# Kaixhin/imitation-learning

Hardware: NVIDIA H100
Metric: env_steps_per_s (higher is better)
Workload: dtype f32

## Files before the change

imitation-learning_b200/csrc/tc_gemm.cu:

```cuda
#include "common.cuh"
#include <cstdio>
#include <cstdlib>

namespace {

constexpr int BM = 128, BN = 256, BK = 16;
constexpr int THREADS = 256;
constexpr int A_BYTES = BM * BK * 4, B_BYTES = BN * BK * 4;
constexpr int A_HI = 0, A_LO = A_BYTES, B_HI = 2 * A_BYTES, B_LO = 2 * A_BYTES + B_BYTES;
constexpr int STAGE_BYTES = 2 * (A_BYTES + B_BYTES);
constexpr int N_STAGES = 3;
constexpr int RAW_STAGES = 3;
constexpr int HEAD_MAX = 8;
constexpr int HEAD_BYTES = (BN + HEAD_MAX * BN) * 4;
constexpr int L1_MAXK = 16, L1_ROWS = 256;
constexpr int L1_W_BYTES = L1_ROWS * L1_MAXK * 4, L1_B_BYTES = L1_ROWS * 4, L1_X_BYTES = BM * L1_MAXK * 4;
constexpr int raw_a_bytes(bool fuse) { return fuse ? 0 : A_BYTES; }
constexpr int raw_bytes(bool fuse) { return raw_a_bytes(fuse) + B_BYTES; }
constexpr int RAW_OFF = N_STAGES * STAGE_BYTES;
constexpr int head_off(bool fuse) { return RAW_OFF + RAW_STAGES * raw_bytes(fuse); }
constexpr int l1_off(bool fuse) { return head_off(fuse) + HEAD_BYTES; }
constexpr int smem_bytes(bool fuse) { return 1024 + l1_off(fuse) + (fuse ? L1_W_BYTES + L1_B_BYTES + L1_X_BYTES : 0); }
static_assert(smem_bytes(false) <= 227 * 1024 && smem_bytes(true) <= 227 * 1024, "tc_gemm: shared memory over the 227 KB per-CTA limit");

__device__ __forceinline__ uint32_t smem_u32(const void* p) { return (uint32_t)__cvta_generic_to_shared(p); }
__device__ __forceinline__ void fence_proxy_async() { asm volatile("fence.proxy.async.shared::cta;" ::: "memory"); }
__device__ __forceinline__ void wgmma_fence() { asm volatile("wgmma.fence.sync.aligned;" ::: "memory"); }
__device__ __forceinline__ void wgmma_commit() { asm volatile("wgmma.commit_group.sync.aligned;" ::: "memory"); }
template <int N>
__device__ __forceinline__ void wgmma_wait() { asm volatile("wgmma.wait_group.sync.aligned %0;" ::"n"(N) : "memory"); }
__device__ __forceinline__ void cp_async16(uint32_t dst, const float* src) { asm volatile("cp.async.cg.shared.global [%0], [%1], 16;" ::"r"(dst), "l"(src) : "memory"); }
__device__ __forceinline__ void cp_async_commit() { asm volatile("cp.async.commit_group;" ::: "memory"); }
template <int N>
__device__ __forceinline__ void cp_async_wait() { asm volatile("cp.async.wait_group %0;" ::"n"(N) : "memory"); }
__device__ __forceinline__ void wgmma_tf32(float (&d)[128], uint64_t a_desc, uint64_t b_desc) {
  asm volatile(
      "wgmma.mma_async.sync.aligned.m64n256k8.f32.tf32.tf32 {"
      "%0, %1, %2, %3, %4, %5, %6, %7, %8, %9, %10, %11, %12, %13, %14, %15, "
      "%16, %17, %18, %19, %20, %21, %22, %23, %24, %25, %26, %27, %28, %29, %30, %31, "
      "%32, %33, %34, %35, %36, %37, %38, %39, %40, %41, %42, %43, %44, %45, %46, %47, "
      "%48, %49, %50, %51, %52, %53, %54, %55, %56, %57, %58, %59, %60, %61, %62, %63, "
      "%64, %65, %66, %67, %68, %69, %70, %71, %72, %73, %74, %75, %76, %77, %78, %79, "
      "%80, %81, %82, %83, %84, %85, %86, %87, %88, %89, %90, %91, %92, %93, %94, %95, "
      "%96, %97, %98, %99, %100, %101, %102, %103, %104, %105, %106, %107, %108, %109, %110, %111, "
      "%112, %113, %114, %115, %116, %117, %118, %119, %120, %121, %122, %123, %124, %125, %126, %127 "
      "}, %128, %129, 1, 1, 1;"
      : "+f"(d[0]), "+f"(d[1]), "+f"(d[2]), "+f"(d[3]), "+f"(d[4]), "+f"(d[5]), "+f"(d[6]), "+f"(d[7]),
        "+f"(d[8]), "+f"(d[9]), "+f"(d[10]), "+f"(d[11]), "+f"(d[12]), "+f"(d[13]), "+f"(d[14]), "+f"(d[15]),
        "+f"(d[16]), "+f"(d[17]), "+f"(d[18]), "+f"(d[19]), "+f"(d[20]), "+f"(d[21]), "+f"(d[22]), "+f"(d[23]),
        "+f"(d[24]), "+f"(d[25]), "+f"(d[26]), "+f"(d[27]), "+f"(d[28]), "+f"(d[29]), "+f"(d[30]), "+f"(d[31]),
        "+f"(d[32]), "+f"(d[33]), "+f"(d[34]), "+f"(d[35]), "+f"(d[36]), "+f"(d[37]), "+f"(d[38]), "+f"(d[39]),
        "+f"(d[40]), "+f"(d[41]), "+f"(d[42]), "+f"(d[43]), "+f"(d[44]), "+f"(d[45]), "+f"(d[46]), "+f"(d[47]),
        "+f"(d[48]), "+f"(d[49]), "+f"(d[50]), "+f"(d[51]), "+f"(d[52]), "+f"(d[53]), "+f"(d[54]), "+f"(d[55]),
        "+f"(d[56]), "+f"(d[57]), "+f"(d[58]), "+f"(d[59]), "+f"(d[60]), "+f"(d[61]), "+f"(d[62]), "+f"(d[63]),
        "+f"(d[64]), "+f"(d[65]), "+f"(d[66]), "+f"(d[67]), "+f"(d[68]), "+f"(d[69]), "+f"(d[70]), "+f"(d[71]),
        "+f"(d[72]), "+f"(d[73]), "+f"(d[74]), "+f"(d[75]), "+f"(d[76]), "+f"(d[77]), "+f"(d[78]), "+f"(d[79]),
        "+f"(d[80]), "+f"(d[81]), "+f"(d[82]), "+f"(d[83]), "+f"(d[84]), "+f"(d[85]), "+f"(d[86]), "+f"(d[87]),
        "+f"(d[88]), "+f"(d[89]), "+f"(d[90]), "+f"(d[91]), "+f"(d[92]), "+f"(d[93]), "+f"(d[94]), "+f"(d[95]),
        "+f"(d[96]), "+f"(d[97]), "+f"(d[98]), "+f"(d[99]), "+f"(d[100]), "+f"(d[101]), "+f"(d[102]), "+f"(d[103]),
        "+f"(d[104]), "+f"(d[105]), "+f"(d[106]), "+f"(d[107]), "+f"(d[108]), "+f"(d[109]), "+f"(d[110]), "+f"(d[111]),
        "+f"(d[112]), "+f"(d[113]), "+f"(d[114]), "+f"(d[115]), "+f"(d[116]), "+f"(d[117]), "+f"(d[118]), "+f"(d[119]),
        "+f"(d[120]), "+f"(d[121]), "+f"(d[122]), "+f"(d[123]), "+f"(d[124]), "+f"(d[125]), "+f"(d[126]), "+f"(d[127])
      : "l"(a_desc), "l"(b_desc));
}
__device__ __forceinline__ uint64_t make_desc(uint32_t smem_addr) {
  return (uint64_t)((smem_addr >> 4) & 0x3FFF) | ((uint64_t)1 << 16) | ((uint64_t)(512 >> 4) << 32) | ((uint64_t)2 << 62);
}
__device__ __forceinline__ uint32_t sw64(int r, int c) { return (uint32_t)((r >> 3) * 512 + (r & 7) * 64 + ((c ^ ((r >> 1) & 3)) << 4)); }
__device__ __forceinline__ void sts128(uint32_t addr, uint32_t x, uint32_t y, uint32_t z, uint32_t w) {
  asm volatile("st.shared.v4.b32 [%0], {%1, %2, %3, %4};" ::"r"(addr), "r"(x), "r"(y), "r"(z), "r"(w) : "memory");
}
__device__ __forceinline__ uint4 lds128(uint32_t addr) {
  uint4 v;
  asm volatile("ld.shared.v4.b32 {%0, %1, %2, %3}, [%4];" : "=r"(v.x), "=r"(v.y), "=r"(v.z), "=r"(v.w) : "r"(addr));
  return v;
}
__device__ __forceinline__ uint32_t hi_of(uint32_t x) { return x & 0xFFFFE000u; }
__device__ __forceinline__ uint32_t lo_of(uint32_t x) { return __float_as_uint(__uint_as_float(x) - __uint_as_float(x & 0xFFFFE000u)); }
__device__ __forceinline__ void store_chunk(uint32_t hi_tile, uint32_t lo_tile, uint32_t off, uint4 v, bool split) {
  sts128(hi_tile + off, hi_of(v.x), hi_of(v.y), hi_of(v.z), hi_of(v.w));
  if (split) sts128(lo_tile + off, lo_of(v.x), lo_of(v.y), lo_of(v.z), lo_of(v.w));
}
__device__ __forceinline__ void store_block_t(uint32_t hi_tile, uint32_t lo_tile, int c4, int kg, const uint4 (&v)[4], bool split) {
  uint4 q0 = make_uint4(v[0].x, v[1].x, v[2].x, v[3].x), q1 = make_uint4(v[0].y, v[1].y, v[2].y, v[3].y);
  uint4 q2 = make_uint4(v[0].z, v[1].z, v[2].z, v[3].z), q3 = make_uint4(v[0].w, v[1].w, v[2].w, v[3].w);
  const int s = (c4 >> 1) & 3;
  if (s & 1) { const uint4 t = q0; q0 = q1; q1 = q2; q2 = q3; q3 = t; }
  if (s & 2) { uint4 t = q0; q0 = q2; q2 = t; t = q1; q1 = q3; q3 = t; }
  store_chunk(hi_tile, lo_tile, sw64(4 * c4 + (s & 3), kg), q0, split);
  store_chunk(hi_tile, lo_tile, sw64(4 * c4 + ((s + 1) & 3), kg), q1, split);
  store_chunk(hi_tile, lo_tile, sw64(4 * c4 + ((s + 2) & 3), kg), q2, split);
  store_chunk(hi_tile, lo_tile, sw64(4 * c4 + ((s + 3) & 3), kg), q3, split);
}

struct TcParams {
  GemmArgs g;
  int tiles_m;
  int split;
  const float* head_w;
  const float* head_b;
  float* head_out;
  int64_t head_gs, head_out_gs;
  int head_n, store_c;
  int head_js, head_ns;
  TcFuseL1 l1;
};

template <int EPI, bool FUSE = false>
__global__ void __launch_bounds__(THREADS, 1) tc_gemm_kernel(const TcParams p) {
  extern __shared__ uint8_t smem_raw[];
  uint8_t* smem = reinterpret_cast<uint8_t*>((reinterpret_cast<uintptr_t>(smem_raw) + 1023) & ~(uintptr_t)1023);
  float* head_s = reinterpret_cast<float*>(smem + head_off(FUSE));
  const uint32_t stage0 = smem_u32(smem), raw0 = stage0 + RAW_OFF;
  const uint32_t w1s = stage0 + l1_off(FUSE), b1s = w1s + L1_W_BYTES, xs = b1s + L1_B_BYTES;
  constexpr uint32_t RAW_A = 0, RAW_B = raw_a_bytes(FUSE), RAW_BYTES = raw_bytes(FUSE);

  const int tid = threadIdx.x, warp = tid >> 5, lane = tid & 31, wg = tid >> 7;
  const GemmArgs& g = p.g;
  const int nkb = g.K / BK, tiles_m = p.tiles_m;
  const int my_tiles = (g.G * tiles_m - (int)blockIdx.x + (int)gridDim.x - 1) / (int)gridDim.x;
  const int nq = my_tiles * nkb;
  const bool a_km = FUSE || g.a_kmajor != 0, b_km = g.b_kmajor != 0, split = p.split != 0;

  const int fr = tid >> 2, fc = tid & 3;
  const int a_c4 = tid & 31, a_kg = (tid >> 5) & 3, b_c4 = tid & 63, b_kg = tid >> 6;
  const uint32_t km_off = sw64(fr, fc);
  auto tile_of = [&](int i) { return (int)blockIdx.x + i * (int)gridDim.x; };

  auto copy_kb = [&](int q) {
    if (q < nq) {
      const int t = tile_of(q / nkb), kb = q % nkb, grp = t / tiles_m, m0 = (t % tiles_m) * BM;
      const uint32_t raw = raw0 + (uint32_t)(q % RAW_STAGES) * RAW_BYTES + (uint32_t)tid * 16u;
      if (!FUSE) {
        const float* A = g.A + (int64_t)(grp / g.a_gdiv) * g.a_gs;
        if (a_km) {
          const float* src = A + (int64_t)(m0 + fr) * g.lda + kb * BK + fc * 4;
          cp_async16(raw + RAW_A, src);
          cp_async16(raw + RAW_A + THREADS * 16, src + (int64_t)64 * g.lda);
        } else if (wg == 0) {
          const float* src = A + (int64_t)(kb * BK + a_kg * 4) * g.lda + m0 + a_c4 * 4;
#pragma unroll
          for (int k = 0; k < 4; ++k) cp_async16(raw + RAW_A + k * (THREADS / 2) * 16, src + (int64_t)k * g.lda);
        }
      }
      const float* Bg = g.B + (int64_t)(grp / g.b_gdiv) * g.b_gs;
      const float* src = b_km ? Bg + (int64_t)fr * g.ldb + kb * BK + fc * 4 : Bg + (int64_t)(kb * BK + b_kg * 4) * g.ldb + b_c4 * 4;
      const int64_t step = b_km ? (int64_t)64 * g.ldb : (int64_t)g.ldb;
#pragma unroll
      for (int j = 0; j < 4; ++j) cp_async16(raw + RAW_B + j * THREADS * 16, src + j * step);
    }
    cp_async_commit();
  };

  auto split_kb = [&](int q) {
    const uint32_t st = stage0 + (uint32_t)(q % N_STAGES) * STAGE_BYTES;
    const uint32_t raw = raw0 + (uint32_t)(q % RAW_STAGES) * RAW_BYTES + (uint32_t)tid * 16u;
    if (FUSE) {
      const int kb = q % nkb, k0 = kb * BK + fc * 4;
      const uint4 bq = lds128(b1s + (uint32_t)k0 * 4u);
      float c0[4] = {__uint_as_float(bq.x), __uint_as_float(bq.y), __uint_as_float(bq.z), __uint_as_float(bq.w)};
      float c1[4] = {c0[0], c0[1], c0[2], c0[3]};
      const int np = (p.l1.x_k + 3) >> 2;
#pragma unroll
      for (int c4 = 0; c4 < L1_MAXK / 4; ++c4) {
        if (c4 < np) {
          const uint4 x0 = lds128(xs + sw64(fr, c4)), x1 = lds128(xs + sw64(fr + 64, c4));
#pragma unroll
          for (int qq = 0; qq < 4; ++qq) {
            const uint4 w = lds128(w1s + (uint32_t)((k0 + qq) * 64 + ((c4 ^ fc) << 4)));
            c0[qq] = fmaf(__uint_as_float(x0.x), __uint_as_float(w.x), c0[qq]); c1[qq] = fmaf(__uint_as_float(x1.x), __uint_as_float(w.x), c1[qq]);
            c0[qq] = fmaf(__uint_as_float(x0.y), __uint_as_float(w.y), c0[qq]); c1[qq] = fmaf(__uint_as_float(x1.y), __uint_as_float(w.y), c1[qq]);
            c0[qq] = fmaf(__uint_as_float(x0.z), __uint_as_float(w.z), c0[qq]); c1[qq] = fmaf(__uint_as_float(x1.z), __uint_as_float(w.z), c1[qq]);
            c0[qq] = fmaf(__uint_as_float(x0.w), __uint_as_float(w.w), c0[qq]); c1[qq] = fmaf(__uint_as_float(x1.w), __uint_as_float(w.w), c1[qq]);
          }
        }
      }
      const uint4 a0 = make_uint4(__float_as_uint(fmaxf(c0[0], 0.f)), __float_as_uint(fmaxf(c0[1], 0.f)), __float_as_uint(fmaxf(c0[2], 0.f)), __float_as_uint(fmaxf(c0[3], 0.f)));
      const uint4 a1 = make_uint4(__float_as_uint(fmaxf(c1[0], 0.f)), __float_as_uint(fmaxf(c1[1], 0.f)), __float_as_uint(fmaxf(c1[2], 0.f)), __float_as_uint(fmaxf(c1[3], 0.f)));
      store_chunk(st + A_HI, st + A_LO, km_off, a0, split);
      store_chunk(st + A_HI, st + A_LO, km_off + 4096u, a1, split);
      if (p.l1.store) {
        const int t = tile_of(q / nkb);
        float* hs = p.l1.store + (int64_t)(t / tiles_m) * p.l1.store_gs + (int64_t)((t % tiles_m) * BM + fr) * g.K + k0;
        *reinterpret_cast<uint4*>(hs) = a0;
        *reinterpret_cast<uint4*>(hs + (int64_t)64 * g.K) = a1;
      }
    } else if (a_km) {
      store_chunk(st + A_HI, st + A_LO, km_off, lds128(raw + RAW_A), split);
      store_chunk(st + A_HI, st + A_LO, km_off + 4096u, lds128(raw + RAW_A + THREADS * 16), split);
    } else if (wg == 0) {
      uint4 v[4];
#pragma unroll
      for (int k = 0; k < 4; ++k) v[k] = lds128(raw + RAW_A + k * (THREADS / 2) * 16);
      store_block_t(st + A_HI, st + A_LO, a_c4, a_kg, v, split);
    }
    if (b_km) {
#pragma unroll
      for (int j = 0; j < 4; ++j) store_chunk(st + B_HI, st + B_LO, km_off + (uint32_t)j * 4096u, lds128(raw + RAW_B + j * THREADS * 16), split);
    } else {
      uint4 v[4];
#pragma unroll
      for (int k = 0; k < 4; ++k) v[k] = lds128(raw + RAW_B + k * THREADS * 16);
      store_block_t(st + B_HI, st + B_LO, b_c4, b_kg, v, split);
    }
  };

  auto stage_l1 = [&](int t) {
    const int grp = t / tiles_m, m0 = (t % tiles_m) * BM, xk = p.l1.x_k;
    const float* w1 = p.l1.w1 + (int64_t)grp * p.l1.gs;
    const float* b1 = p.l1.b1 + (int64_t)grp * p.l1.gs;
    const float* x = p.l1.x + (int64_t)(grp / p.l1.x_gdiv) * p.l1.x_gs + (int64_t)m0 * p.l1.x_ld;
    float* w1f = reinterpret_cast<float*>(smem + l1_off(FUSE));
    float* b1f = reinterpret_cast<float*>(smem + l1_off(FUSE) + L1_W_BYTES);
    float* xf = reinterpret_cast<float*>(smem + l1_off(FUSE) + L1_W_BYTES + L1_B_BYTES);
    for (int i = tid; i < L1_ROWS * L1_MAXK; i += THREADS) {
      const int k = i / L1_MAXK, j = i % L1_MAXK;
      w1f[k * L1_MAXK + ((((j >> 2) ^ ((k >> 2) & 3)) << 2) | (j & 3))] = (k < g.K && j < xk) ? __ldg(w1 + (int64_t)k * xk + j) : 0.f;
    }
    for (int i = tid; i < L1_ROWS; i += THREADS) b1f[i] = i < g.K ? __ldg(b1 + i) : 0.f;
    for (int i = tid; i < BM * L1_MAXK; i += THREADS) {
      const int r = i / L1_MAXK, j = i % L1_MAXK;
      xf[(sw64(r, j >> 2) >> 2) + (j & 3)] = j < xk ? __ldg(x + (int64_t)r * p.l1.x_ld + j) : 0.f;
    }
  };

#pragma unroll 1
  for (int q = 0; q < RAW_STAGES; ++q) copy_kb(q);
  if (FUSE) {
    stage_l1(tile_of(0));
    __syncthreads();
  }
  cp_async_wait<RAW_STAGES - 1>();
  split_kb(0);
  copy_kb(RAW_STAGES);
  fence_proxy_async();
  __syncthreads();
  const uint64_t a_desc0 = make_desc(stage0 + (uint32_t)wg * 4096u), b_desc0 = make_desc(stage0);

  float acc[128];
#pragma unroll 1
  for (int i = 0, q = 0; i < my_tiles; ++i) {
#pragma unroll
    for (int j = 0; j < 128; ++j) acc[j] = 0.f;
#pragma unroll 1
    for (int kb = 0; kb < nkb; ++kb, ++q) {
      const uint32_t cur = (uint32_t)(q % N_STAGES) * STAGE_BYTES;
      wgmma_fence();
#pragma unroll
      for (int kk = 0; kk < BK / 8; ++kk) {
        const uint32_t o = cur + kk * 32;
        const uint64_t ah = a_desc0 + ((o + A_HI) >> 4), al = a_desc0 + ((o + A_LO) >> 4), bh = b_desc0 + ((o + B_HI) >> 4), bl = b_desc0 + ((o + B_LO) >> 4);
        if (split) {
          wgmma_tf32(acc, al, bh);
          wgmma_tf32(acc, ah, bl);
        }
        wgmma_tf32(acc, ah, bh);
      }
      wgmma_commit();
      if (q + 1 < nq) {
        if (FUSE && kb == nkb - 1) {
          stage_l1(tile_of(i + 1));
          __syncthreads();
        }
        cp_async_wait<RAW_STAGES - 1>();
        split_kb(q + 1);
      }
      copy_kb(q + 1 + RAW_STAGES);
      wgmma_wait<1>();
      fence_proxy_async();
      __syncthreads();
    }

    const int t = tile_of(i), grp = t / tiles_m, m0 = (t % tiles_m) * BM;
    if (EPI == 4 || EPI == 6) {
      const float* wsrc = p.head_w + (int64_t)grp * p.head_gs;
      if (EPI == 4) head_s[tid] = __ldg(g.bias + (int64_t)grp * g.bias_gs + tid);
#pragma unroll
      for (int j = 0; j < HEAD_MAX; ++j)
        if (j < p.head_n) head_s[BN + j * BN + tid] = __ldg(wsrc + (int64_t)j * p.head_js + (int64_t)tid * p.head_ns);
    }
    wgmma_wait<0>();
    if (EPI == 4 || EPI == 6) __syncthreads();
    const int r0 = m0 + wg * 64 + (warp & 3) * 16 + (lane >> 2), cl = (lane & 3) * 2;
    float* C = g.C + (int64_t)grp * g.c_gs + (int64_t)r0 * g.ldc + cl;
    const int64_t c8 = (int64_t)8 * g.ldc;
    const float* bias = (EPI == 1 || (EPI == 3 && g.bias)) ? g.bias + (int64_t)grp * g.bias_gs + cl : nullptr;
    const float* mask = (EPI == 2 || (EPI == 3 && g.mask)) ? g.mask + (int64_t)grp * g.mask_gs + (int64_t)r0 * g.ldmask + cl : nullptr;
    const int64_t m8 = (int64_t)8 * g.ldmask;
    const uint32_t* mbits = (EPI == 5 || EPI == 6) ? g.mask_bits + (int64_t)grp * g.mask_bits_gs + (int64_t)r0 * (BN / 32) : nullptr;
    uint32_t word0 = 0, word1 = 0;
#pragma unroll
    for (int c = 0; c < BN / 8; ++c) {
      float v00 = acc[4 * c], v01 = acc[4 * c + 1], v10 = acc[4 * c + 2], v11 = acc[4 * c + 3];
      const int col = 8 * c, bit = (c & 3) * 8 + cl;
      if (EPI == 5 || EPI == 6) {
        if ((c & 3) == 0) { word0 = __ldg(mbits + (c >> 2)); word1 = __ldg(mbits + 8 * (BN / 32) + (c >> 2)); }
        v00 = (word0 >> bit) & 1u ? v00 : 0.f; v01 = (word0 >> (bit + 1)) & 1u ? v01 : 0.f;
        v10 = (word1 >> bit) & 1u ? v10 : 0.f; v11 = (word1 >> (bit + 1)) & 1u ? v11 : 0.f;
      }
      if (EPI == 4) {
        const float2 b = *reinterpret_cast<const float2*>(head_s + col + cl);
        v00 = fmaxf(v00 + b.x, 0.f); v01 = fmaxf(v01 + b.y, 0.f); v10 = fmaxf(v10 + b.x, 0.f); v11 = fmaxf(v11 + b.y, 0.f);
        if (g.bits_out) {
          if ((c & 3) == 0) word0 = word1 = 0;
          word0 |= (v00 > 0.f ? 1u : 0u) << bit | (v01 > 0.f ? 1u : 0u) << (bit + 1);
          word1 |= (v10 > 0.f ? 1u : 0u) << bit | (v11 > 0.f ? 1u : 0u) << (bit + 1);
          if ((c & 3) == 3) {
            word0 |= __shfl_xor_sync(0xffffffffu, word0, 1); word0 |= __shfl_xor_sync(0xffffffffu, word0, 2);
            word1 |= __shfl_xor_sync(0xffffffffu, word1, 1); word1 |= __shfl_xor_sync(0xffffffffu, word1, 2);
            if ((lane & 3) == 0) {
              uint32_t* bo = g.bits_out + (int64_t)grp * g.bits_out_gs + (int64_t)r0 * (BN / 32) + (c >> 2);
              bo[0] = word0;
              bo[8 * (BN / 32)] = word1;
            }
          }
        }
      }
      if (EPI == 4 || EPI == 6) {
        acc[4 * c] = v00; acc[4 * c + 1] = v01; acc[4 * c + 2] = v10; acc[4 * c + 3] = v11;
        if (!p.store_c) continue;
      }
      if (EPI == 1) {
        const float2 b = __ldg(reinterpret_cast<const float2*>(bias + col));
        v00 = fmaxf(v00 + b.x, 0.f); v01 = fmaxf(v01 + b.y, 0.f); v10 = fmaxf(v10 + b.x, 0.f); v11 = fmaxf(v11 + b.y, 0.f);
      } else if (EPI == 2) {
        const float2 ma = __ldg(reinterpret_cast<const float2*>(mask + col)), mb = __ldg(reinterpret_cast<const float2*>(mask + m8 + col));
        v00 = ma.x > 0.f ? v00 : 0.f; v01 = ma.y > 0.f ? v01 : 0.f; v10 = mb.x > 0.f ? v10 : 0.f; v11 = mb.y > 0.f ? v11 : 0.f;
      } else if (EPI == 3) {
        if (bias) {
          const float2 b = __ldg(reinterpret_cast<const float2*>(bias + col));
          v00 += b.x; v01 += b.y; v10 += b.x; v11 += b.y;
        }
        if (g.act >= 0) { v00 = act_apply(v00, g.act); v01 = act_apply(v01, g.act); v10 = act_apply(v10, g.act); v11 = act_apply(v11, g.act); }
        if (mask) {
          const float2 ma = __ldg(reinterpret_cast<const float2*>(mask + col)), mb = __ldg(reinterpret_cast<const float2*>(mask + m8 + col));
          v00 *= act_grad_from_output(ma.x, g.mask_act); v01 *= act_grad_from_output(ma.y, g.mask_act);
          v10 *= act_grad_from_output(mb.x, g.mask_act); v11 *= act_grad_from_output(mb.y, g.mask_act);
        }
      }
      *reinterpret_cast<float2*>(C + col) = make_float2(v00, v01);
      *reinterpret_cast<float2*>(C + c8 + col) = make_float2(v10, v11);
    }
    if (EPI == 4 || EPI == 6) {
      float* ho = p.head_out + (int64_t)grp * p.head_out_gs + (int64_t)r0 * p.head_n;
      const float* hb = p.head_b ? p.head_b + (int64_t)grp * p.head_gs : nullptr;
#pragma unroll 1
      for (int j = 0; j < HEAD_MAX; ++j) {
        if (j < p.head_n) {
          float s0 = 0.f, s1 = 0.f;
#pragma unroll
          for (int c = 0; c < BN / 8; ++c) {
            const float2 w = *reinterpret_cast<const float2*>(head_s + BN + j * BN + 8 * c + cl);
            s0 = fmaf(acc[4 * c], w.x, s0); s0 = fmaf(acc[4 * c + 1], w.y, s0);
            s1 = fmaf(acc[4 * c + 2], w.x, s1); s1 = fmaf(acc[4 * c + 3], w.y, s1);
          }
          s0 += __shfl_xor_sync(0xffffffffu, s0, 1); s0 += __shfl_xor_sync(0xffffffffu, s0, 2);
          s1 += __shfl_xor_sync(0xffffffffu, s1, 1); s1 += __shfl_xor_sync(0xffffffffu, s1, 2);
          if ((lane & 3) == 0) {
            const float b = hb ? __ldg(hb + j) : 0.f;
            ho[j] = s0 + b;
            ho[(int64_t)8 * p.head_n + j] = s1 + b;
          }
        }
      }
    }
  }
  cp_async_wait<0>();
}

__global__ void colsum_kernel(const float* __restrict__ A, int64_t a_gs, int a_gdiv, int lda, int K, int M, float* __restrict__ out, int64_t out_gs) {
  const int g = blockIdx.y, m = blockIdx.x * blockDim.x + threadIdx.x;
  if (m >= M) return;
  const float* a = A + (int64_t)(g / a_gdiv) * a_gs + m;
  float s = 0.f;
  for (int k = 0; k < K; ++k) s += a[(int64_t)k * lda];
  out[(int64_t)g * out_gs + m] = s;
}

}

bool tc_gemm_eligible(const GemmArgs& a) {
  auto al16 = [](const void* p) { return (reinterpret_cast<uintptr_t>(p) & 15) == 0; };
  if (a.M % BM != 0 || a.N != BN || a.K % BK != 0 || a.accumulate) return false;
  if (a.a_kmajor == 0 && a.b_kmajor != 0) return false;
  if (!al16(a.A) || !al16(a.B) || !al16(a.C) || a.lda % 4 || a.ldb % 4 || a.ldc % 4 || a.a_gs % 4 || a.b_gs % 4 || a.c_gs % 4) return false;
  if (a.bias && (!al16(a.bias) || a.bias_gs % 4)) return false;
  if (a.mask && (!al16(a.mask) || a.ldmask % 4 || a.mask_gs % 4)) return false;
  return true;
}

template <int EPI, bool FUSE = false>
int tc_set_attr() {
  IL_CUDA(cudaFuncSetAttribute(tc_gemm_kernel<EPI, FUSE>, cudaFuncAttributeMaxDynamicSharedMemorySize, smem_bytes(FUSE)));
  return 0;
}

int tc_gemm_init() {
  IL_TRY((tc_set_attr<0>())); IL_TRY((tc_set_attr<1>())); IL_TRY((tc_set_attr<2>())); IL_TRY((tc_set_attr<3>())); IL_TRY((tc_set_attr<4>()));
  IL_TRY((tc_set_attr<4, true>())); IL_TRY((tc_set_attr<5>())); IL_TRY((tc_set_attr<6>()));
  return 0;
}

template <int EPI, bool FUSE = false>
static int tc_launch(il_handle* h, TcParams& p, cudaStream_t stream) {
  const GemmArgs& a = p.g;
  p.tiles_m = a.M / BM;
  const int tiles = a.G * p.tiles_m, wave = h->sm_count >= p.tiles_m ? h->sm_count / p.tiles_m * p.tiles_m : h->sm_count;
  IL_LAUNCH(h, (tc_gemm_kernel<EPI, FUSE>), tiles < wave ? tiles : wave, THREADS, smem_bytes(FUSE), stream, p);
  return 0;
}

bool tc_head_fusable(const il_handle* h, const GemmArgs& a, int head_n) {
  return h->gemm_mode != IL_GEMM_FP32 && tc_gemm_eligible(a) && a.bias && a.act == IL_ACT_RELU && !a.mask && !a.colsum && head_n >= 1 && head_n <= HEAD_MAX;
}

bool tc_l1_fusable(const il_handle* h, const GemmArgs& a, int x_k) {
  return h->tc_fuse_l1 && tc_gemm_eligible(a) && x_k >= 1 && x_k <= L1_MAXK && a.K <= L1_ROWS && a.a_kmajor;
}

int launch_tc_gemm_head(il_handle* h, const GemmArgs& a, const float* head_w, const float* head_b, int64_t head_gs, int head_n, float* head_out, int64_t head_out_gs, int store_c,
                        cudaStream_t stream, const TcFuseL1* l1) {
  IL_CHECK(tc_head_fusable(h, a, head_n), "tc_gemm_head: not fusable");
  TcParams p{};
  p.g = a;
  p.split = h->gemm_mode == IL_GEMM_TF32X3 ? 1 : 0;
  p.head_w = head_w; p.head_b = head_b; p.head_out = head_out; p.head_gs = head_gs; p.head_out_gs = head_out_gs; p.head_n = head_n; p.store_c = store_c;
  p.head_js = BN; p.head_ns = 1;
  double bytes = gemm_algorithmic_bytes(a, store_c != 0) + 4.0 * a.G * (double)a.M * head_n, flops = 2.0 * a.M * a.N * a.K * a.G;
  if (l1) {
    IL_CHECK(tc_l1_fusable(h, a, l1->x_k), "tc_gemm_head: first layer not fusable (K0=%d)", l1->x_k);
    IL_CHECK(l1->x && l1->w1 && l1->b1 && (reinterpret_cast<uintptr_t>(l1->b1) & 15) == 0 && l1->gs % 4 == 0, "tc_gemm_head: bad first-layer buffers");
    IL_CHECK(!l1->store || ((reinterpret_cast<uintptr_t>(l1->store) & 15) == 0 && l1->store_gs % 4 == 0), "tc_gemm_head: unaligned hidden store");
    p.l1 = *l1;
    const double gx = (a.G + l1->x_gdiv - 1) / l1->x_gdiv;
    bytes += -4.0 * a.G * (double)a.M * a.K + 4.0 * (gx * a.M * l1->x_k + (double)a.G * a.K * (l1->x_k + 1)) + (l1->store ? 4.0 * a.G * (double)a.M * a.K : 0.0);
    flops += 2.0 * a.G * (double)a.M * a.K * l1->x_k;
  }
  auto run = [&]() { return l1 ? tc_launch<4, true>(h, p, stream) : tc_launch<4>(h, p, stream); };
  if (h->profiling) {
    ProfiledLaunch pl;
    IL_TRY(profile_open(h, &pl, flops, bytes, stream));
    const int rc = run();
    IL_TRY(profile_close(h, &pl, stream));
    return rc;
  }
  return run();
}

bool tc_dx_head_fusable(const il_handle* h, const GemmArgs& a, int head_n) {
  return h->gemm_mode != IL_GEMM_FP32 && a.M >= 128 && a.K >= 128 && tc_gemm_eligible(a) && a.mask_bits && !a.mask && !a.bias && a.act < 0 && !a.colsum && a.mask_act == IL_ACT_RELU &&
         head_n >= 1 && head_n <= HEAD_MAX;
}
int launch_tc_gemm_dx_head(il_handle* h, const GemmArgs& a, const float* w, int64_t w_gs, int w_ns, int head_n, float* out, int64_t out_gs, cudaStream_t stream) {
  IL_CHECK(tc_dx_head_fusable(h, a, head_n), "tc_gemm_dx_head: not fusable");
  TcParams p{};
  p.g = a;
  p.split = h->gemm_mode == IL_GEMM_TF32X3 ? 1 : 0;
  p.head_w = w; p.head_b = nullptr; p.head_out = out; p.head_gs = w_gs; p.head_out_gs = out_gs; p.head_n = head_n; p.store_c = 0;
  p.head_js = 1; p.head_ns = w_ns;
  const double bytes = gemm_algorithmic_bytes(a, false) + 4.0 * a.G * (double)a.M * head_n, flops = 2.0 * a.M * a.N * a.K * a.G;
  if (h->profiling) {
    ProfiledLaunch pl;
    IL_TRY(profile_open(h, &pl, flops, bytes, stream));
    const int rc = tc_launch<6>(h, p, stream);
    IL_TRY(profile_close(h, &pl, stream));
    return rc;
  }
  return tc_launch<6>(h, p, stream);
}

int launch_tc_gemm(il_handle* h, const GemmArgs& a, cudaStream_t stream) {
  IL_CHECK(tc_gemm_eligible(a), "tc_gemm: shape/layout not eligible (M=%d N=%d K=%d)", a.M, a.N, a.K);
  TcParams p{};
  p.g = a;
  p.split = h->gemm_mode == IL_GEMM_TF32X3 ? 1 : 0;
  const bool bits = a.mask_bits != nullptr;
  IL_CHECK(!bits || (!a.bias && a.act < 0 && a.mask_act == IL_ACT_RELU), "tc_gemm: sign-bit masks are the ReLU derivative of a plain product");
  if (bits) p.g.mask = nullptr;
  const bool plain = !a.bias && a.act < 0 && !a.mask && !bits;
  const bool bias_relu = a.bias && a.act == IL_ACT_RELU && !a.mask;
  const bool mask_relu = !a.bias && a.act < 0 && a.mask && a.mask_act == IL_ACT_RELU && !bits;
  if (bits) IL_TRY(tc_launch<5>(h, p, stream));
  else if (plain) IL_TRY(tc_launch<0>(h, p, stream));
  else if (bias_relu) IL_TRY(tc_launch<1>(h, p, stream));
  else if (mask_relu) IL_TRY(tc_launch<2>(h, p, stream));
  else IL_TRY(tc_launch<3>(h, p, stream));
  if (a.colsum) {
    dim3 cg((a.M + 127) / 128, a.G);
    IL_LAUNCH(h, colsum_kernel, cg, 128, 0, stream, a.A, a.a_gs, a.a_gdiv, a.lda, a.K, a.M, a.colsum, a.colsum_gs);
  }
  return 0;
}
```

Baseline: 79460.

## Warp-specialize TF32 wgmma GEMM into producer and consumer warpgroups with mbarriers

Splits the CTA into a 128-thread producer warpgroup, which runs the cp.async loads, the hi/lo split, the fused L1 staging and smem layout conversion, and two consumer warpgroups that issue wgmma and run the epilogue. Full/empty mbarriers replace the per-k-block __syncthreads, and setmaxnreg moves registers from the producer to the consumers. The goal is to overlap the split/convert work with tensor-core math and to drop block-wide barriers. In exchange the producer has half as many threads for the split work, and the extra synchronization adds complexity and risks deadlock or ordering bugs.

```diff
diff --git a/imitation-learning_b200/csrc/tc_gemm.cu b/imitation-learning_b200/csrc/tc_gemm.cu
--- a/imitation-learning_b200/csrc/tc_gemm.cu
+++ b/imitation-learning_b200/csrc/tc_gemm.cu
@@ -5,7 +5,13 @@
 namespace {
 
 constexpr int BM = 128, BN = 256, BK = 16;
-constexpr int THREADS = 256;
+constexpr int PRODUCER_THREADS = 128, CONSUMER_THREADS = 256;
+constexpr int THREADS = PRODUCER_THREADS + CONSUMER_THREADS;
+constexpr int LAUNCH_REGS = 168;
+constexpr int producer_regs(bool fuse) { return fuse ? 72 : 56; }
+constexpr int consumer_regs(bool fuse) { return (THREADS * LAUNCH_REGS - PRODUCER_THREADS * producer_regs(fuse)) / CONSUMER_THREADS; }
+static_assert(THREADS * LAUNCH_REGS <= 65536 && consumer_regs(false) % 8 == 0 && consumer_regs(true) % 8 == 0, "tc_gemm: setmaxnreg split");
+constexpr int CONSUMER_BAR = 1, PRODUCER_BAR = 2;
 constexpr int A_BYTES = BM * BK * 4, B_BYTES = BN * BK * 4;
 constexpr int A_HI = 0, A_LO = A_BYTES, B_HI = 2 * A_BYTES, B_LO = 2 * A_BYTES + B_BYTES;
 constexpr int STAGE_BYTES = 2 * (A_BYTES + B_BYTES);
@@ -20,6 +26,8 @@
 constexpr int RAW_OFF = N_STAGES * STAGE_BYTES;
 constexpr int head_off(bool fuse) { return RAW_OFF + RAW_STAGES * raw_bytes(fuse); }
 constexpr int l1_off(bool fuse) { return head_off(fuse) + HEAD_BYTES; }
+constexpr int BAR_BYTES = 64;
+static_assert(2 * N_STAGES * 8 <= BAR_BYTES && BAR_BYTES + 512 - 16 <= 1024, "tc_gemm: mbarrier area");
 constexpr int smem_bytes(bool fuse) { return 1024 + l1_off(fuse) + (fuse ? L1_W_BYTES + L1_B_BYTES + L1_X_BYTES : 0); }
 static_assert(smem_bytes(false) <= 227 * 1024 && smem_bytes(true) <= 227 * 1024, "tc_gemm: shared memory over the 227 KB per-CTA limit");
 
@@ -33,6 +41,20 @@
 __device__ __forceinline__ void cp_async_commit() { asm volatile("cp.async.commit_group;" ::: "memory"); }
 template <int N>
 __device__ __forceinline__ void cp_async_wait() { asm volatile("cp.async.wait_group %0;" ::"n"(N) : "memory"); }
+__device__ __forceinline__ void mbar_init(uint32_t bar, uint32_t count) { asm volatile("mbarrier.init.shared::cta.b64 [%0], %1;" ::"r"(bar), "r"(count) : "memory"); }
+__device__ __forceinline__ void mbar_arrive(uint32_t bar) { asm volatile("mbarrier.arrive.shared::cta.b64 _, [%0];" ::"r"(bar) : "memory"); }
+__device__ __forceinline__ void mbar_wait(uint32_t bar, uint32_t parity) {
+  asm volatile(
+      "{\n .reg .pred p;\n"
+      "WAIT:\n mbarrier.try_wait.parity.shared::cta.b64 p, [%0], %1;\n"
+      " @!p bra WAIT;\n}" ::"r"(bar), "r"(parity) : "memory");
+}
+template <int ID, int N>
+__device__ __forceinline__ void named_bar_sync() { asm volatile("bar.sync %0, %1;" ::"n"(ID), "n"(N) : "memory"); }
+template <int R>
+__device__ __forceinline__ void setmaxnreg_dec() { asm volatile("setmaxnreg.dec.sync.aligned.u32 %0;" ::"n"(R)); }
+template <int R>
+__device__ __forceinline__ void setmaxnreg_inc() { asm volatile("setmaxnreg.inc.sync.aligned.u32 %0;" ::"n"(R)); }
 __device__ __forceinline__ void wgmma_tf32(float (&d)[128], uint64_t a_desc, uint64_t b_desc) {
   asm volatile(
       "wgmma.mma_async.sync.aligned.m64n256k8.f32.tf32.tf32 {"
@@ -109,9 +131,10 @@
 template <int EPI, bool FUSE = false>
 __global__ void __launch_bounds__(THREADS, 1) tc_gemm_kernel(const TcParams p) {
   extern __shared__ uint8_t smem_raw[];
-  uint8_t* smem = reinterpret_cast<uint8_t*>((reinterpret_cast<uintptr_t>(smem_raw) + 1023) & ~(uintptr_t)1023);
+  uint8_t* smem = reinterpret_cast<uint8_t*>((reinterpret_cast<uintptr_t>(smem_raw) + BAR_BYTES + 511) & ~(uintptr_t)511);
   float* head_s = reinterpret_cast<float*>(smem + head_off(FUSE));
   const uint32_t stage0 = smem_u32(smem), raw0 = stage0 + RAW_OFF;
+  const uint32_t full0 = stage0 - BAR_BYTES, empty0 = full0 + N_STAGES * 8;
   const uint32_t w1s = stage0 + l1_off(FUSE), b1s = w1s + L1_W_BYTES, xs = b1s + L1_B_BYTES;
   constexpr uint32_t RAW_A = 0, RAW_B = raw_a_bytes(FUSE), RAW_BYTES = raw_bytes(FUSE);
 
@@ -120,131 +143,170 @@
   const int nkb = g.K / BK, tiles_m = p.tiles_m;
   const int my_tiles = (g.G * tiles_m - (int)blockIdx.x + (int)gridDim.x - 1) / (int)gridDim.x;
   const int nq = my_tiles * nkb;
-  const bool a_km = FUSE || g.a_kmajor != 0, b_km = g.b_kmajor != 0, split = p.split != 0;
-
-  const int fr = tid >> 2, fc = tid & 3;
-  const int a_c4 = tid & 31, a_kg = (tid >> 5) & 3, b_c4 = tid & 63, b_kg = tid >> 6;
-  const uint32_t km_off = sw64(fr, fc);
   auto tile_of = [&](int i) { return (int)blockIdx.x + i * (int)gridDim.x; };
 
-  auto copy_kb = [&](int q) {
-    if (q < nq) {
-      const int t = tile_of(q / nkb), kb = q % nkb, grp = t / tiles_m, m0 = (t % tiles_m) * BM;
-      const uint32_t raw = raw0 + (uint32_t)(q % RAW_STAGES) * RAW_BYTES + (uint32_t)tid * 16u;
-      if (!FUSE) {
+  if (tid == 0) {
+#pragma unroll
+    for (int s = 0; s < N_STAGES; ++s) {
+      mbar_init(full0 + 8 * s, PRODUCER_THREADS);
+      mbar_init(empty0 + 8 * s, CONSUMER_THREADS);
+    }
+  }
+  __syncthreads();
+
+  if (wg == 0) {
+    setmaxnreg_dec<producer_regs(FUSE)>();
+    const bool a_km = FUSE || g.a_kmajor != 0, b_km = g.b_kmajor != 0, split = p.split != 0;
+    constexpr int MAP = 2 * PRODUCER_THREADS;
+    const int pt = tid;
+
+    auto copy_kb = [&](int q) {
+      if (q < nq) {
+        const int t = tile_of(q / nkb), kb = q % nkb, grp = t / tiles_m, m0 = (t % tiles_m) * BM;
         const float* A = g.A + (int64_t)(grp / g.a_gdiv) * g.a_gs;
-        if (a_km) {
-          const float* src = A + (int64_t)(m0 + fr) * g.lda + kb * BK + fc * 4;
-          cp_async16(raw + RAW_A, src);
-          cp_async16(raw + RAW_A + THREADS * 16, src + (int64_t)64 * g.lda);
-        } else if (wg == 0) {
-          const float* src = A + (int64_t)(kb * BK + a_kg * 4) * g.lda + m0 + a_c4 * 4;
-#pragma unroll
-          for (int k = 0; k < 4; ++k) cp_async16(raw + RAW_A + k * (THREADS / 2) * 16, src + (int64_t)k * g.lda);
-        }
-      }
-      const float* Bg = g.B + (int64_t)(grp / g.b_gdiv) * g.b_gs;
-      const float* src = b_km ? Bg + (int64_t)fr * g.ldb + kb * BK + fc * 4 : Bg + (int64_t)(kb * BK + b_kg * 4) * g.ldb + b_c4 * 4;
-      const int64_t step = b_km ? (int64_t)64 * g.ldb : (int64_t)g.ldb;
-#pragma unroll
-      for (int j = 0; j < 4; ++j) cp_async16(raw + RAW_B + j * THREADS * 16, src + j * step);
+        const float* Bg = g.B + (int64_t)(grp / g.b_gdiv) * g.b_gs;
+#pragma unroll
+        for (int h = 0; h < 2; ++h) {
+          const int v = pt + h * PRODUCER_THREADS, fr = v >> 2, fc = v & 3;
+          const uint32_t raw = raw0 + (uint32_t)(q % RAW_STAGES) * RAW_BYTES + (uint32_t)v * 16u;
+          if (!FUSE) {
+            if (a_km) {
+              const float* src = A + (int64_t)(m0 + fr) * g.lda + kb * BK + fc * 4;
+              cp_async16(raw + RAW_A, src);
+              cp_async16(raw + RAW_A + MAP * 16, src + (int64_t)64 * g.lda);
+            } else if (h == 0) {
+              const float* src = A + (int64_t)(kb * BK + ((v >> 5) & 3) * 4) * g.lda + m0 + (v & 31) * 4;
+#pragma unroll
+              for (int k = 0; k < 4; ++k) cp_async16(raw + RAW_A + k * (MAP / 2) * 16, src + (int64_t)k * g.lda);
+            }
+          }
+          const float* src = b_km ? Bg + (int64_t)fr * g.ldb + kb * BK + fc * 4 : Bg + (int64_t)(kb * BK + (v >> 6) * 4) * g.ldb + (v & 63) * 4;
+          const int64_t step = b_km ? (int64_t)64 * g.ldb : (int64_t)g.ldb;
+#pragma unroll
+          for (int j = 0; j < 4; ++j) cp_async16(raw + RAW_B + j * MAP * 16, src + j * step);
+        }
+      }
+      cp_async_commit();
+    };
+
+    auto split_kb = [&](int q, int s) {
+      const uint32_t st = stage0 + (uint32_t)s * STAGE_BYTES;
+#pragma unroll(FUSE ? 1 : 2)
+      for (int h = 0; h < 2; ++h) {
+        const int v = pt + h * PRODUCER_THREADS, fr = v >> 2, fc = v & 3;
+        const uint32_t raw = raw0 + (uint32_t)(q % RAW_STAGES) * RAW_BYTES + (uint32_t)v * 16u;
+        const uint32_t km_off = sw64(fr, fc);
+        if (FUSE) {
+          const int kb = q % nkb, k0 = kb * BK + fc * 4;
+          const uint4 bq = lds128(b1s + (uint32_t)k0 * 4u);
+          float c0[4] = {__uint_as_float(bq.x), __uint_as_float(bq.y), __uint_as_float(bq.z), __uint_as_float(bq.w)};
+          float c1[4] = {c0[0], c0[1], c0[2], c0[3]};
+          const int np = (p.l1.x_k + 3) >> 2;
+#pragma unroll
+          for (int c4 = 0; c4 < L1_MAXK / 4; ++c4) {
+            if (c4 < np) {
+              const uint4 x0 = lds128(xs + sw64(fr, c4)), x1 = lds128(xs + sw64(fr + 64, c4));
+#pragma unroll
+              for (int qq = 0; qq < 4; ++qq) {
+                const uint4 w = lds128(w1s + (uint32_t)((k0 + qq) * 64 + ((c4 ^ fc) << 4)));
+                c0[qq] = fmaf(__uint_as_float(x0.x), __uint_as_float(w.x), c0[qq]); c1[qq] = fmaf(__uint_as_float(x1.x), __uint_as_float(w.x), c1[qq]);
+                c0[qq] = fmaf(__uint_as_float(x0.y), __uint_as_float(w.y), c0[qq]); c1[qq] = fmaf(__uint_as_float(x1.y), __uint_as_float(w.y), c1[qq]);
+                c0[qq] = fmaf(__uint_as_float(x0.z), __uint_as_float(w.z), c0[qq]); c1[qq] = fmaf(__uint_as_float(x1.z), __uint_as_float(w.z), c1[qq]);
+                c0[qq] = fmaf(__uint_as_float(x0.w), __uint_as_float(w.w), c0[qq]); c1[qq] = fmaf(__uint_as_float(x1.w), __uint_as_float(w.w), c1[qq]);
+              }
+            }
+          }
+          const uint4 a0 = make_uint4(__float_as_uint(fmaxf(c0[0], 0.f)), __float_as_uint(fmaxf(c0[1], 0.f)), __float_as_uint(fmaxf(c0[2], 0.f)), __float_as_uint(fmaxf(c0[3], 0.f)));
+          const uint4 a1 = make_uint4(__float_as_uint(fmaxf(c1[0], 0.f)), __float_as_uint(fmaxf(c1[1], 0.f)), __float_as_uint(fmaxf(c1[2], 0.f)), __float_as_uint(fmaxf(c1[3], 0.f)));
+          store_chunk(st + A_HI, st + A_LO, km_off, a0, split);
+          store_chunk(st + A_HI, st + A_LO, km_off + 4096u, a1, split);
+          if (p.l1.store) {
+            const int t = tile_of(q / nkb);
+            float* hs = p.l1.store + (int64_t)(t / tiles_m) * p.l1.store_gs + (int64_t)((t % tiles_m) * BM + fr) * g.K + k0;
+            *reinterpret_cast<uint4*>(hs) = a0;
+            *reinterpret_cast<uint4*>(hs + (int64_t)64 * g.K) = a1;
+          }
+        } else if (a_km) {
+          store_chunk(st + A_HI, st + A_LO, km_off, lds128(raw + RAW_A), split);
+          store_chunk(st + A_HI, st + A_LO, km_off + 4096u, lds128(raw + RAW_A + MAP * 16), split);
+        } else if (h == 0) {
+          uint4 va[4];
+#pragma unroll
+          for (int k = 0; k < 4; ++k) va[k] = lds128(raw + RAW_A + k * (MAP / 2) * 16);
+          store_block_t(st + A_HI, st + A_LO, v & 31, (v >> 5) & 3, va, split);
+        }
+        if (b_km) {
+#pragma unroll
+          for (int j = 0; j < 4; ++j) store_chunk(st + B_HI, st + B_LO, km_off + (uint32_t)j * 4096u, lds128(raw + RAW_B + j * MAP * 16), split);
+        } else {
+          uint4 vb[4];
+#pragma unroll
+          for (int k = 0; k < 4; ++k) vb[k] = lds128(raw + RAW_B + k * MAP * 16);
+          store_block_t(st + B_HI, st + B_LO, v & 63, v >> 6, vb, split);
+        }
+      }
+    };
+
+    auto stage_l1 = [&](int t) {
+      const int grp = t / tiles_m, m0 = (t % tiles_m) * BM, xk = p.l1.x_k;
+      const float* w1 = p.l1.w1 + (int64_t)grp * p.l1.gs;
+      const float* b1 = p.l1.b1 + (int64_t)grp * p.l1.gs;
+      const float* x = p.l1.x + (int64_t)(grp / p.l1.x_gdiv) * p.l1.x_gs + (int64_t)m0 * p.l1.x_ld;
+      float* w1f = reinterpret_cast<float*>(smem + l1_off(FUSE));
+      float* b1f = reinterpret_cast<float*>(smem + l1_off(FUSE) + L1_W_BYTES);
+      float* xf = reinterpret_cast<float*>(smem + l1_off(FUSE) + L1_W_BYTES + L1_B_BYTES);
+#pragma unroll 1
+      for (int i = pt; i < L1_ROWS * L1_MAXK; i += PRODUCER_THREADS) {
+        const int k = i / L1_MAXK, j = i % L1_MAXK;
+        w1f[k * L1_MAXK + ((((j >> 2) ^ ((k >> 2) & 3)) << 2) | (j & 3))] = (k < g.K && j < xk) ? __ldg(w1 + (int64_t)k * xk + j) : 0.f;
+      }
+      for (int i = pt; i < L1_ROWS; i += PRODUCER_THREADS) b1f[i] = i < g.K ? __ldg(b1 + i) : 0.f;
+#pragma unroll 1
+      for (int i = pt; i < BM * L1_MAXK; i += PRODUCER_THREADS) {
+        const int r = i / L1_MAXK, j = i % L1_MAXK;
+        xf[(sw64(r, j >> 2) >> 2) + (j & 3)] = j < xk ? __ldg(x + (int64_t)r * p.l1.x_ld + j) : 0.f;
+      }
+    };
+
+#pragma unroll 1
+    for (int q = 0; q < RAW_STAGES; ++q) copy_kb(q);
+    int s = 0;
+    uint32_t ph = 1;
+#pragma unroll 1
+    for (int q = 0; q < nq; ++q) {
+      if (FUSE && q % nkb == 0) {
+        if (q > 0) named_bar_sync<PRODUCER_BAR, PRODUCER_THREADS>();
+        stage_l1(tile_of(q / nkb));
+        named_bar_sync<PRODUCER_BAR, PRODUCER_THREADS>();
+      }
+      mbar_wait(empty0 + 8 * s, ph);
+      cp_async_wait<RAW_STAGES - 1>();
+      split_kb(q, s);
+      fence_proxy_async();
+      mbar_arrive(full0 + 8 * s);
+      copy_kb(q + RAW_STAGES);
+      if (++s == N_STAGES) { s = 0; ph ^= 1; }
     }
-    cp_async_commit();
-  };
-
-  auto split_kb = [&](int q) {
-    const uint32_t st = stage0 + (uint32_t)(q % N_STAGES) * STAGE_BYTES;
-    const uint32_t raw = raw0 + (uint32_t)(q % RAW_STAGES) * RAW_BYTES + (uint32_t)tid * 16u;
-    if (FUSE) {
-      const int kb = q % nkb, k0 = kb * BK + fc * 4;
-      const uint4 bq = lds128(b1s + (uint32_t)k0 * 4u);
-      float c0[4] = {__uint_as_float(bq.x), __uint_as_float(bq.y), __uint_as_float(bq.z), __uint_as_float(bq.w)};
-      float c1[4] = {c0[0], c0[1], c0[2], c0[3]};
-      const int np = (p.l1.x_k + 3) >> 2;
-#pragma unroll
-      for (int c4 = 0; c4 < L1_MAXK / 4; ++c4) {
-        if (c4 < np) {
-          const uint4 x0 = lds128(xs + sw64(fr, c4)), x1 = lds128(xs + sw64(fr + 64, c4));
-#pragma unroll
-          for (int qq = 0; qq < 4; ++qq) {
-            const uint4 w = lds128(w1s + (uint32_t)((k0 + qq) * 64 + ((c4 ^ fc) << 4)));
-            c0[qq] = fmaf(__uint_as_float(x0.x), __uint_as_float(w.x), c0[qq]); c1[qq] = fmaf(__uint_as_float(x1.x), __uint_as_float(w.x), c1[qq]);
-            c0[qq] = fmaf(__uint_as_float(x0.y), __uint_as_float(w.y), c0[qq]); c1[qq] = fmaf(__uint_as_float(x1.y), __uint_as_float(w.y), c1[qq]);
-            c0[qq] = fmaf(__uint_as_float(x0.z), __uint_as_float(w.z), c0[qq]); c1[qq] = fmaf(__uint_as_float(x1.z), __uint_as_float(w.z), c1[qq]);
-            c0[qq] = fmaf(__uint_as_float(x0.w), __uint_as_float(w.w), c0[qq]); c1[qq] = fmaf(__uint_as_float(x1.w), __uint_as_float(w.w), c1[qq]);
-          }
-        }
-      }
-      const uint4 a0 = make_uint4(__float_as_uint(fmaxf(c0[0], 0.f)), __float_as_uint(fmaxf(c0[1], 0.f)), __float_as_uint(fmaxf(c0[2], 0.f)), __float_as_uint(fmaxf(c0[3], 0.f)));
-      const uint4 a1 = make_uint4(__float_as_uint(fmaxf(c1[0], 0.f)), __float_as_uint(fmaxf(c1[1], 0.f)), __float_as_uint(fmaxf(c1[2], 0.f)), __float_as_uint(fmaxf(c1[3], 0.f)));
-      store_chunk(st + A_HI, st + A_LO, km_off, a0, split);
-      store_chunk(st + A_HI, st + A_LO, km_off + 4096u, a1, split);
-      if (p.l1.store) {
-        const int t = tile_of(q / nkb);
-        float* hs = p.l1.store + (int64_t)(t / tiles_m) * p.l1.store_gs + (int64_t)((t % tiles_m) * BM + fr) * g.K + k0;
-        *reinterpret_cast<uint4*>(hs) = a0;
-        *reinterpret_cast<uint4*>(hs + (int64_t)64 * g.K) = a1;
-      }
-    } else if (a_km) {
-      store_chunk(st + A_HI, st + A_LO, km_off, lds128(raw + RAW_A), split);
-      store_chunk(st + A_HI, st + A_LO, km_off + 4096u, lds128(raw + RAW_A + THREADS * 16), split);
-    } else if (wg == 0) {
-      uint4 v[4];
-#pragma unroll
-      for (int k = 0; k < 4; ++k) v[k] = lds128(raw + RAW_A + k * (THREADS / 2) * 16);
-      store_block_t(st + A_HI, st + A_LO, a_c4, a_kg, v, split);
-    }
-    if (b_km) {
-#pragma unroll
-      for (int j = 0; j < 4; ++j) store_chunk(st + B_HI, st + B_LO, km_off + (uint32_t)j * 4096u, lds128(raw + RAW_B + j * THREADS * 16), split);
-    } else {
-      uint4 v[4];
-#pragma unroll
-      for (int k = 0; k < 4; ++k) v[k] = lds128(raw + RAW_B + k * THREADS * 16);
-      store_block_t(st + B_HI, st + B_LO, b_c4, b_kg, v, split);
-    }
-  };
-
-  auto stage_l1 = [&](int t) {
-    const int grp = t / tiles_m, m0 = (t % tiles_m) * BM, xk = p.l1.x_k;
-    const float* w1 = p.l1.w1 + (int64_t)grp * p.l1.gs;
-    const float* b1 = p.l1.b1 + (int64_t)grp * p.l1.gs;
-    const float* x = p.l1.x + (int64_t)(grp / p.l1.x_gdiv) * p.l1.x_gs + (int64_t)m0 * p.l1.x_ld;
-    float* w1f = reinterpret_cast<float*>(smem + l1_off(FUSE));
-    float* b1f = reinterpret_cast<float*>(smem + l1_off(FUSE) + L1_W_BYTES);
-    float* xf = reinterpret_cast<float*>(smem + l1_off(FUSE) + L1_W_BYTES + L1_B_BYTES);
-    for (int i = tid; i < L1_ROWS * L1_MAXK; i += THREADS) {
-      const int k = i / L1_MAXK, j = i % L1_MAXK;
-      w1f[k * L1_MAXK + ((((j >> 2) ^ ((k >> 2) & 3)) << 2) | (j & 3))] = (k < g.K && j < xk) ? __ldg(w1 + (int64_t)k * xk + j) : 0.f;
-    }
-    for (int i = tid; i < L1_ROWS; i += THREADS) b1f[i] = i < g.K ? __ldg(b1 + i) : 0.f;
-    for (int i = tid; i < BM * L1_MAXK; i += THREADS) {
-      const int r = i / L1_MAXK, j = i % L1_MAXK;
-      xf[(sw64(r, j >> 2) >> 2) + (j & 3)] = j < xk ? __ldg(x + (int64_t)r * p.l1.x_ld + j) : 0.f;
-    }
-  };
-
-#pragma unroll 1
-  for (int q = 0; q < RAW_STAGES; ++q) copy_kb(q);
-  if (FUSE) {
-    stage_l1(tile_of(0));
-    __syncthreads();
-  }
-  cp_async_wait<RAW_STAGES - 1>();
-  split_kb(0);
-  copy_kb(RAW_STAGES);
-  fence_proxy_async();
-  __syncthreads();
-  const uint64_t a_desc0 = make_desc(stage0 + (uint32_t)wg * 4096u), b_desc0 = make_desc(stage0);
-
+    cp_async_wait<0>();
+    return;
+  }
+
+  setmaxnreg_inc<consumer_regs(FUSE)>();
+  const int cw = wg - 1, ct = tid - PRODUCER_THREADS;
+  const uint64_t a_desc0 = make_desc(stage0 + (uint32_t)cw * 4096u), b_desc0 = make_desc(stage0);
+  const bool split = p.split != 0;
   float acc[128];
-#pragma unroll 1
-  for (int i = 0, q = 0; i < my_tiles; ++i) {
+  int s = 0;
+  uint32_t ph = 0;
+#pragma unroll 1
+  for (int i = 0; i < my_tiles; ++i) {
 #pragma unroll
     for (int j = 0; j < 128; ++j) acc[j] = 0.f;
-#pragma unroll 1
-    for (int kb = 0; kb < nkb; ++kb, ++q) {
-      const uint32_t cur = (uint32_t)(q % N_STAGES) * STAGE_BYTES;
+    int prev = 0;
+#pragma unroll 1
+    for (int kb = 0; kb < nkb; ++kb) {
+      mbar_wait(full0 + 8 * s, ph);
+      const uint32_t cur = (uint32_t)s * STAGE_BYTES;
       wgmma_fence();
 #pragma unroll
       for (int kk = 0; kk < BK / 8; ++kk) {
@@ -257,31 +319,25 @@
         wgmma_tf32(acc, ah, bh);
       }
       wgmma_commit();
-      if (q + 1 < nq) {
-        if (FUSE && kb == nkb - 1) {
-          stage_l1(tile_of(i + 1));
-          __syncthreads();
-        }
-        cp_async_wait<RAW_STAGES - 1>();
-        split_kb(q + 1);
-      }
-      copy_kb(q + 1 + RAW_STAGES);
       wgmma_wait<1>();
-      fence_proxy_async();
-      __syncthreads();
+      if (kb > 0) mbar_arrive(empty0 + 8 * prev);
+      prev = s;
+      if (++s == N_STAGES) { s = 0; ph ^= 1; }
     }
 
     const int t = tile_of(i), grp = t / tiles_m, m0 = (t % tiles_m) * BM;
     if (EPI == 4 || EPI == 6) {
+      named_bar_sync<CONSUMER_BAR, CONSUMER_THREADS>();
       const float* wsrc = p.head_w + (int64_t)grp * p.head_gs;
-      if (EPI == 4) head_s[tid] = __ldg(g.bias + (int64_t)grp * g.bias_gs + tid);
+      if (EPI == 4) head_s[ct] = __ldg(g.bias + (int64_t)grp * g.bias_gs + ct);
 #pragma unroll
       for (int j = 0; j < HEAD_MAX; ++j)
-        if (j < p.head_n) head_s[BN + j * BN + tid] = __ldg(wsrc + (int64_t)j * p.head_js + (int64_t)tid * p.head_ns);
+        if (j < p.head_n) head_s[BN + j * BN + ct] = __ldg(wsrc + (int64_t)j * p.head_js + (int64_t)ct * p.head_ns);
     }
     wgmma_wait<0>();
-    if (EPI == 4 || EPI == 6) __syncthreads();
-    const int r0 = m0 + wg * 64 + (warp & 3) * 16 + (lane >> 2), cl = (lane & 3) * 2;
+    mbar_arrive(empty0 + 8 * prev);
+    if (EPI == 4 || EPI == 6) named_bar_sync<CONSUMER_BAR, CONSUMER_THREADS>();
+    const int r0 = m0 + cw * 64 + (warp & 3) * 16 + (lane >> 2), cl = (lane & 3) * 2;
     float* C = g.C + (int64_t)grp * g.c_gs + (int64_t)r0 * g.ldc + cl;
     const int64_t c8 = (int64_t)8 * g.ldc;
     const float* bias = (EPI == 1 || (EPI == 3 && g.bias)) ? g.bias + (int64_t)grp * g.bias_gs + cl : nullptr;
@@ -365,8 +421,8 @@
       }
     }
   }
-  cp_async_wait<0>();
-}
+}
+
 
 __global__ void colsum_kernel(const float* __restrict__ A, int64_t a_gs, int a_gdiv, int lda, int K, int M, float* __restrict__ out, int64_t out_gs) {
   const int g = blockIdx.y, m = blockIdx.x * blockDim.x + threadIdx.x;
```

After: 82360 (median of 6 runs). +3.7%, better.
